# davnords/octic-vits

Measured on AMD Instinct MI355X. Metric: images/sec Hybrid Octic ViT-H/14 224² bf16 train step @1/2/4/8 MI355X, higher is better.
Workload: dtype bf16; 1 GPU; hybrid_deit_huge_patch14 (16 octic + 16 standard blocks, drop_path 0.5) DeiT-III train step: bf16-autocast fwd + bwd + LAMB + EMA, 224x224, batch 64/GPU (BASELINE configs[1]), data parallel over 1 GPU(s); global_batch=64, per_gpu_batch=64, accum_steps=1, parallelism=dp1, library_gemm_table=True, launch=hipGraph replay (whole step)

## Files before the change

include/octic_hip.h:

```cpp
#ifndef OCTIC_HIP_H
#define OCTIC_HIP_H

#include <stdint.h>

#ifdef __cplusplus
extern "C" {
#endif

#define OCTIC_ABI_VERSION 20

enum { OCTIC_F32 = 0, OCTIC_BF16 = 1, OCTIC_U8 = 2  };

enum {
  OCTIC_OK = 0,
  OCTIC_ESHAPE = -1,
  OCTIC_EALIGN = -2,
  OCTIC_EDTYPE = -3,
  OCTIC_ENULL = -4,
  OCTIC_EWORKSPACE = -5
};

typedef struct {
  void* ptr[5];
  int64_t ld[5];
// ... 100 lines not shown
int octic_linear_d8_ring_order_dropped(int ngroups, const int* items, const int* ksteps, int slots_per_xcd, const int* n_chunks,
                                       const unsigned char* dead_long, const unsigned char* dead_short, int* out_group,
                                       int* out_item, int* out_dead);

int octic_linear_d8_wgrad_has_colsum(int cin, int cout, int dtype);
enum {
  OCTIC_WGRAD_RING = 0,
  OCTIC_WGRAD_TILED = 1
};
int octic_linear_d8_wgrad_plan(int64_t M, int cin, int cout, int dtype, int out[4]);
int64_t octic_linear_d8_wgrad_workspace_bytes(int cin, int cout, int splits);
int octic_linear_d8_wgrad_splits(int64_t M, int cin, int cout);
int octic_linear_d8_wgrad_tile(int64_t M, int cin, int cout);
int octic_linear_d8_wgrad(const octic_view* x, const octic_view* dy, int64_t M, int cin, int cout, int dtype,
                          float* workspace, int splits, void* stream);
int octic_linear_d8_wgrad_finish(const float* workspace, int splits, int cin, int cout,
                                 const float* const w32[5], const float* const cs[5], const float* bias,
                                 const float* dysum, float* const dw[5], float* const dcs[5], float* dbias,
                                 void* stream);
typedef struct octic_wgrad_finish_job {
  const float* workspace;
  const float* w32[5];
  const float* cs[5];
  const float* bias;
  const float* dysum;
  float* dw[5];
  float* dcs[5];
  float* dbias;
  int splits, cin, cout, has_cs;
} octic_wgrad_finish_job;
// ... 448 lines not shown
```

octic_vits_amd/_lib.py:

```python
import ctypes
import os
import re

HERE = os.path.dirname(os.path.abspath(__file__))
LIB_PATH = os.environ.get("OCTIC_LIB") or os.path.join(HERE, "liboctic_hip.so")
HEADER_PATH = os.path.join(HERE, "..", "include", "octic_hip.h")

F32, BF16, U8 = 0, 1, 2
ABI_VERSION = 20
(ROUTE_DENSE_TILE, ROUTE_DENSE_SPLIT, ROUTE_WGRAD_SLABS, ROUTE_WGRAD_TILE, ROUTE_LINEAR_RING, ROUTE_RING_EVEN,
 ROUTE_ATTN_LEGACY, ROUTE_ATTN_ONLINE, ROUTE_ATTN_BWD_PAIR, ROUTE_DENSE_IMAGE, ROUTE_DENSE_CLS2, ROUTE_ATTN_STREAM) = range(12)

DENSE_ADAPT_WIDE, DENSE_ADAPT_NARROW = 16, 32
DENSE_IMAGE_ALWAYS, DENSE_IMAGE_CLS_APART, DENSE_IMAGE_NEVER = 4, 8, 16

(ATTN_FWD_PERSIST, ATTN_FWD_A80_ONESHOT, ATTN_FWD_A80_ONLINE, ATTN_FWD_RESIDENT, ATTN_FWD_STREAM, ATTN_FWD_F32) = range(6)
ATTN_BWD_SINGLE, ATTN_BWD_PAIR, ATTN_BWD_STREAM, ATTN_BWD_F32 = range(4)
LINEAR_WREG, LINEAR_RING, LINEAR_CLASSIC = range(3)
WGRAD_RING, WGRAD_TILED = range(2)
DENSE_F32_NT, DENSE_F32_NN, DENSE_F32_TN = range(3)

c_i64, c_int, c_float, c_void_p = ctypes.c_int64, ctypes.c_int, ctypes.c_float, ctypes.c_void_p
c_double = ctypes.c_double

# ... 31 lines not shown
    "octic_linear_d8_fwd": (c_int, [VP, c_void_p, c_void_p, VP, VP, c_void_p, c_i64, c_void_p, c_i64, c_int, c_int,
                                    c_int, c_int, c_void_p]),
    "octic_linear_d8_fwd_skip": (c_int, [VP, c_void_p, c_void_p, VP, VP, c_void_p, c_i64, c_void_p, c_i64, c_int, c_int,
                                         c_int, c_int, c_void_p, c_i64, c_void_p]),
    "octic_linear_d8_fwd_dropped": (c_int, [VP, c_void_p, c_void_p, VP, VP, c_void_p, c_i64, c_void_p, c_i64, c_int, c_int,
                                            c_int, c_int, c_void_p, c_i64, c_void_p]),
    "octic_linear_d8_tile_n": (c_int, [c_i64, c_int, c_int]),
    "octic_linear_d8_plan": (c_int, [c_i64, c_int, c_int, c_int, c_int, c_int, ctypes.POINTER(c_int)]),
    "octic_linear_d8_ring_order": (c_int, [c_void_p, c_void_p, c_void_p, c_int, c_void_p, c_void_p]),
    "octic_linear_d8_ring_order_dropped": (c_int, [c_int, c_void_p, c_void_p, c_int, c_void_p, c_void_p, c_void_p, c_void_p,
                                                   c_void_p, c_void_p]),
    "octic_linear_d8_wgrad_tile": (c_int, [c_i64, c_int, c_int]),
    "octic_linear_d8_wgrad_workspace_bytes": (c_i64, [c_int, c_int, c_int]),
    "octic_linear_d8_wgrad_splits": (c_int, [c_i64, c_int, c_int]),
    "octic_linear_d8_wgrad": (c_int, [VP, VP, c_i64, c_int, c_int, c_int, c_void_p, c_int, c_void_p]),
    "octic_linear_d8_wgrad_finish": (c_int, [c_void_p, c_int, c_int, c_int, c_void_p, c_void_p, c_void_p, c_void_p,
                                             c_void_p, c_void_p, c_void_p, c_void_p]),
    "octic_linear_d8_wgrad_finish_batch": (c_int, [c_void_p, c_int, c_void_p]),
    "octic_linear_d8_wgrad_has_colsum": (c_int, [c_int, c_int, c_int]),
    "octic_linear_d8_wgrad_plan": (c_int, [c_i64, c_int, c_int, c_int, ctypes.POINTER(c_int)]),
    "octic_lamb_workspace_floats": (c_i64, [c_int, c_int]),
    "octic_lamb_step": (c_int, [c_void_p] * 10 + [c_int, c_int, c_void_p, c_float, c_float, c_float, c_float, c_float,
                                                  c_int, c_float, c_void_p, c_void_p]),
    "octic_adamw_step": (c_int, [c_void_p] * 10 + [c_int, c_int, c_void_p, c_float, c_float, c_float, c_float, c_float,
                                                   c_int, c_float, c_void_p, c_void_p]),
    "octic_lamb_step_hp": (c_int, [c_void_p] * 10 + [c_int, c_int, c_void_p, c_void_p, c_float, c_float, c_float, c_float,
                                                     c_int, c_void_p, c_void_p, c_void_p]),
    "octic_adamw_step_hp": (c_int, [c_void_p] * 10 + [c_int, c_int, c_void_p, c_void_p, c_float, c_float, c_float, c_float,
                                                      c_int, c_void_p, c_void_p, c_void_p]),
    "octic_dense_blocks": (c_int, [c_i64]),
# ... 283 lines not shown
```

octic_vits_amd/csrc/wgrad.hip:

```cpp
#include <stdlib.h>
#include "octic_common.hpp"

namespace octic {

struct WgGroup {
  const char* x;
  int64_t x_ld;
  const char* dy;
  int64_t dy_ld;
  int64_t rows;
  int K, N;
  int pair;
  int k_tiles, n_tiles;
  int wg_begin;
  int splits;
  int64_t slab_off;
  float* colsum;
};
struct WgArgs {
  WgGroup g[5];
  int ngroups;
  int wgs;
  int64_t slab_elems;
  float* slabs;
};

template <typename T> struct WElem;
template <> struct WElem<float> { static constexpr int EPC = 4; static constexpr int BMR = 32; };
template <> struct WElem<bf16> { static constexpr int EPC = 8; static constexpr int BMR = 64; };

template <typename TIN, int TT>
__global__ __launch_bounds__(256) void wgrad_kernel(WgArgs args) {
  constexpr int EPC = WElem<TIN>::EPC;
  constexpr int BMR = WElem<TIN>::BMR;
  constexpr int BW = 32 * TT;
  constexpr int CPR = BW / EPC;
  constexpr int RS = BW * (int)sizeof(TIN) + 16;
  constexpr int TILE = BMR * RS;
  extern __shared__ __attribute__((aligned(16))) char lds[];
// ... 135 lines not shown
#ifndef OCTIC_WG_STAGES
#define OCTIC_WG_STAGES 3
#endif
constexpr int kWgS = OCTIC_WG_STAGES, kWgR = 32;
constexpr int kWgTile = kWgR * 320;
constexpr int kWgStage = 2 * kWgTile;
__device__ __attribute__((aligned(256))) unsigned char g_wg_zero[512];

__device__ inline void wg_wait_tiles(int ahead) {
  if (ahead <= 0) asm volatile("s_waitcnt vmcnt(0)" ::: "memory");
  else if (ahead == 1) asm volatile("s_waitcnt vmcnt(5)" ::: "memory");
  else if (ahead == 2) asm volatile("s_waitcnt vmcnt(10)" ::: "memory");
  else asm volatile("s_waitcnt vmcnt(15)" ::: "memory");
}

__global__ __launch_bounds__(256, 2) void wgrad_ring_kernel(WgArgs args) {
  constexpr int TT = 5, BW = 160;
  extern __shared__ __attribute__((aligned(16))) char lds[];
  const int nwg = gridDim.x, bid = blockIdx.x;
  const int xcd = bid & 7, q8 = nwg >> 3, r8 = nwg & 7;
  const int lid = (xcd < r8 ? xcd * (q8 + 1) : r8 * (q8 + 1) + (xcd - r8) * q8) + (bid >> 3);
  int gi = 0;
#pragma unroll
  for (int i = 1; i < 5; ++i)
    if (i < args.ngroups && lid >= args.g[i].wg_begin) gi = i;
  const WgGroup& G = args.g[gi];
  const int gt = G.k_tiles * G.n_tiles;
  const int rel = lid - G.wg_begin;
  const int split = rel / gt, lt = rel - split * gt;
  const int kt = lt / G.n_tiles, nt = lt - kt * G.n_tiles;
  const int k0 = kt * BW, n0 = nt * BW;
  const int K = G.K, N = G.N;
  int64_t chunk = (G.rows + G.splits - 1) / G.splits;
  chunk = (chunk + kWgR - 1) / kWgR * kWgR;
  const int64_t r0 = (int64_t)split * chunk;
  const int64_t r1 = r0 + chunk < G.rows ? r0 + chunk : G.rows;
  const int nsteps = r0 < r1 ? (int)((r1 - r0 + kWgR - 1) / kWgR) : 0;

  const int tid = threadIdx.x, lane = tid & 63, wid = tid >> 6;
  const int wk = wid & 1, wn = wid >> 1;
  const int fr = lane & 15, kg = lane >> 4;

  const char* src[5];
  int64_t inc[5];
  int row_in_tile[5], cbyte[5], ldst[5];
#pragma unroll
  for (int j = 0; j < 5; ++j) {
    const int q = wid + 4 * j;
    const bool isY = q >= 10;
    const int qq = isY ? q - 10 : q;
    const int o = qq * 1024 + lane * 16;
    const int row = o / 320;
    const int cpos = (o - row * 320) >> 4;
    const int c = ((row & 8) ? cpos + 18 : cpos) % 20;
    const int64_t mm = r0 + row;
    const int64_t ld = isY ? G.dy_ld : G.x_ld;
    const int width = isY ? N : K;
    const int64_t ro = G.pair ? (mm >> 1) * ld + (mm & 1) * (int64_t)width : mm * ld;
    src[j] = (isY ? G.dy : G.x) + (ro + (isY ? n0 : k0)) * 2 + c * 16;
    inc[j] = (G.pair ? 16 : 32) * ld * 2;
    row_in_tile[j] = row;
    cbyte[j] = c * 16;
    ldst[j] = (isY ? kWgTile : 0) + qq * 1024;
  }
  int l_step = 0, l_stage = 0;
  auto issue = [&]() {
    const unsigned st = lds_offset(lds) + l_stage * kWgStage;
    const bool tail = (int64_t)(l_step + 1) * kWgR > r1 - r0;
#pragma unroll
    for (int j = 0; j < 5; ++j) {
      const char* p = src[j];
      if (tail && r0 + (int64_t)l_step * kWgR + row_in_tile[j] >= r1) p = (const char*)g_wg_zero + cbyte[j];
      dma16_to_lds(st + ldst[j], p);
      src[j] += inc[j];
    }
    l_stage = l_stage == kWgS - 1 ? 0 : l_stage + 1;
    ++l_step;
  };

  f32x4 acc[TT][TT];
#pragma unroll
  for (int i = 0; i < TT; ++i)
#pragma unroll
    for (int j = 0; j < TT; ++j) acc[i][j] = f32x4{0, 0, 0, 0};
  const bool do_cs = G.colsum != nullptr && kt == 0 && wk == 0;
  f32x4 accs[TT];
#pragma unroll
  for (int j = 0; j < TT; ++j) accs[j] = f32x4{0, 0, 0, 0};
  const bf16 one = (bf16)1.0f;
  const bf16x8 ones = {one, one, one, one, one, one, one, one};

  const int frow = kg * 8 + (fr >> 2);
  const int rot = (kg & 1) * 2;
  int offa[TT], offb[TT];
#pragma unroll
  for (int i = 0; i < TT; ++i) {
    const int ca = wk * 10 + i * 2 + ((fr & 3) >> 1), cb = wn * 10 + i * 2 + ((fr & 3) >> 1);
    offa[i] = frow * 320 + ((ca + rot) % 20) * 16 + (fr & 1) * 8;
    offb[i] = kWgTile + frow * 320 + ((cb + rot) % 20) * 16 + (fr & 1) * 8;
  }

#pragma unroll
  for (int pz = 0; pz < kWgS - 1; ++pz)
    if (pz < nsteps) issue();
  int c_stage = 0;
  for (int sidx = 0; sidx < nsteps; ++sidx) {
    const int left = nsteps - 1 - sidx;
    wg_wait_tiles(left < kWgS - 2 ? left : kWgS - 2);
    __builtin_amdgcn_s_barrier();
    if (sidx + kWgS - 1 < nsteps) issue();
    const char* base = lds + c_stage * kWgStage;
    c_stage = c_stage == kWgS - 1 ? 0 : c_stage + 1;
    typedef __attribute__((ext_vector_type(8))) short s16x8;
    bf16x8 af[TT], bfr[TT];
#pragma unroll
    for (int i = 0; i < TT; ++i) {
// ... 144 lines not shown
    a.g[i].n_tiles = (a.g[i].N + BW - 1) / BW;
    a.g[i].wg_begin = t;
    t += a.g[i].k_tiles * a.g[i].n_tiles * a.g[i].splits;
  }
  a.wgs = t;
  constexpr size_t smem = (size_t)2 * 2 * WElem<TIN>::BMR * (BW * sizeof(TIN) + 16);
  static DeviceOnce once;
  if (once.first()) {
    (void)hipFuncSetAttribute((const void*)wgrad_kernel<TIN, TT>, hipFuncAttributeMaxDynamicSharedMemorySize, (int)smem);
    (void)hipGetLastError();
  }
  wgrad_kernel<TIN, TT><<<t, 256, smem, s>>>(a);
  return launch_status();
}

inline int launch_wgrad_ring(WgArgs& a, hipStream_t s) {
  int t = 0;
  for (int i = 0; i < a.ngroups; ++i) {
    a.g[i].k_tiles = a.g[i].K / 160;
    a.g[i].n_tiles = a.g[i].N / 160;
    a.g[i].wg_begin = t;
    t += a.g[i].k_tiles * a.g[i].n_tiles * a.g[i].splits;
  }
  a.wgs = t;
  static DeviceOnce once;
  if (kWgS * kWgStage > 64 * 1024 && once.first()) {
    (void)hipFuncSetAttribute((const void*)wgrad_ring_kernel, hipFuncAttributeMaxDynamicSharedMemorySize, kWgS * kWgStage);
    (void)hipGetLastError();
  }
  wgrad_ring_kernel<<<t, 256, kWgS * kWgStage, s>>>(a);
  return launch_status();
}

#ifndef OCTIC_WG_TARGET
#define OCTIC_WG_TARGET 512.0
#endif
struct WgPlan {
  int kernel;
  int tt;
  int splits;
};
inline WgPlan wgrad_plan(const WgArgs& a, int dtype) {
  WgPlan p = {dtype == OCTIC_BF16 ? OCTIC_WGRAD_RING : OCTIC_WGRAD_TILED, pick_tt(a), 1};
  for (int i = 0; i < a.ngroups; ++i)
    if ((a.g[i].K % 160) || (a.g[i].N % 160)) p.kernel = OCTIC_WGRAD_TILED;
// ... 50 lines not shown
}

int octic_linear_d8_wgrad_has_colsum(int cin, int cout, int dtype) {
  int out[4];
  return octic_linear_d8_wgrad_plan(1, cin, cout, dtype, out) == OCTIC_OK && out[3];
}
int octic_linear_d8_wgrad_tile(int64_t M, int cin, int cout) {
  int out[4];
  return octic_linear_d8_wgrad_plan(M, cin, cout, OCTIC_F32, out) == OCTIC_OK ? out[1] : 0;
}
int octic_linear_d8_wgrad_splits(int64_t M, int cin, int cout) {
  int out[4];
  return octic_linear_d8_wgrad_plan(M, cin, cout, OCTIC_F32, out) == OCTIC_OK ? out[2] : 1;
}

int octic_linear_d8_wgrad(const octic_view* x, const octic_view* dy, int64_t M, int cin, int cout, int dtype,
                          float* workspace, int splits, void* stream) {
  int e;
  if ((e = check_c_dt(cin, dtype)) || (e = check_c_dt(cout, dtype))) return e;
  if ((e = check_view(x, cin, dtype)) || (e = check_view(dy, cout, dtype))) return e;
  if (!workspace) return OCTIC_ENULL;
  if (M <= 0 || splits <= 0) return OCTIC_ESHAPE;
  WgArgs a = {};
  a.slab_elems = linear_slab_elems(cin, cout);
  a.slabs = workspace;
  d8_group_table(a, M, cin, cout);
  for (int gidx = 0; gidx < 5; ++gidx) {
    const int irrep = d8_group_irrep(gidx);
    const bool isE = irrep == 4;
    WgGroup& g = a.g[gidx];
    g.x = (const char*)x->ptr[irrep];
    g.x_ld = x->ld[irrep];
    g.dy = (const char*)dy->ptr[irrep];
    g.dy_ld = dy->ld[irrep];
    g.splits = group_splits(splits, isE);
    g.slab_off = isE ? (int64_t)4 * cin * cout : (int64_t)irrep * cin * cout;
    g.colsum = irrep == 0 ? workspace + colsum_off_elems(cin, cout, splits) : nullptr;
  }
  if (dtype == OCTIC_F32) return launch_wgrad<float>(a, (hipStream_t)stream);
  if (dtype == OCTIC_BF16) return launch_wgrad<bf16>(a, (hipStream_t)stream);
// ... 108 lines not shown
```

octic_vits_amd/d8_layers.py:

```python
import collections.abc
import math
from itertools import repeat

import torch
import torch.nn as nn
import torch.nn.functional as F

from . import functional as OF
from .d8_utils import SQRT2, SQRT2_OVER_4, convert_5tuple_to_8tuple, convert_8tuple_to_5tuple, expand_lift_kernel, packed_lift_weight
from .functional import Octic, as_packed, compute_dtype


def _ntuple(n):
    def parse(x):
        if isinstance(x, collections.abc.Iterable) and not isinstance(x, str):
            return tuple(x)
        return tuple(repeat(x, n))
    return parse


to_2tuple = _ntuple(2)

drop_path_mask_source = None

# ... 204 lines not shown
        if input_channels % 8 != 0 or output_channels % 8 != 0:
            raise ValueError()
        self.bias = bias
        self.input_channels, self.output_channels = input_channels, output_channels
        ci, co = input_channels // 8, output_channels // 8
        self.lin_A1 = nn.Linear(ci, co, bias=bias)
        self.lin_A2 = nn.Linear(ci, co, bias=False)
        self.lin_B1 = nn.Linear(ci, co, bias=False)
        self.lin_B2 = nn.Linear(ci, co, bias=False)
        self.lin_E = nn.Linear(2 * ci, 2 * co, bias=False)
        self._prep = OF.WeightPrep()

    def weights(self):
        return tuple(getattr(self, "lin_" + n).weight for n in _IRREPS)

    def forward(self, x_batched, resid=None, rs=None, cs=None, next_norm=None, skip_out=None, skip_dx=None, zero_dx=None):
        assert len(x_batched) == 5, "Input should be a 5-tuple"
        xp, cin = as_packed(x_batched)
        if 8 * cin != self.input_channels:
            raise ValueError(f"LinearD8: expected {self.input_channels} channels, got {8 * cin}")
        cout = self.output_channels // 8
        dtype = compute_dtype(xp)
        rps = xp.shape[-2] if xp.dim() >= 2 else 1
        if rs is not None and rs.numel() == xp.numel() // xp.shape[-1] and rs.numel() != xp.shape[0]:
            rps = 1
        cs5 = (None,) * 5 if cs is None else tuple(cs)
        if torch.compiler.is_compiling():
            from . import dispatch as _D
            xq = xp if xp.dtype == dtype else xp.to(dtype)
            fl = self._prep.flat if dtype == torch.bfloat16 else None
            pwb, pwt = fl if fl is not None else (None, None)
            y = torch.ops.octic.linear_d8(xq, *self.weights(), self.lin_A1.bias, resid, rs, *cs5, cin, cout, rps, pwb, pwt)
            return Octic(y, cout) if next_norm is None else (Octic(y, cout), None)
        if (next_norm is not None and resid is not None and OF.OCTIC_NEXT_NORM and xp.is_cuda and dtype == torch.bfloat16
                and resid.dtype == torch.float32 and type(next_norm) is LayerNormD8):
            a, beta = next_norm.affine()
            y, yn = OF.LinearD8NormFn.apply(xp, *self.weights(), self.lin_A1.bias, resid, rs, *cs5, cin, cout, rps, dtype,
                                            self._prep, *a, beta, next_norm.eps, skip_dx)
            return Octic(y, cout), Octic(yn, cout)
        y = OF.LinearD8Fn.apply(xp, *self.weights(), self.lin_A1.bias, resid, rs, *cs5, cin, cout, rps, dtype, self._prep,
                                skip_out, skip_dx, zero_dx)
        return Octic(y, cout) if next_norm is None else (Octic(y, cout), None)

    def extra_repr(self) -> str:
        return f"in_features={self.input_channels}, out_features={self.output_channels}, bias={self.bias is not None}"


class AffineD8(nn.Module):

    def __init__(self, dim, bias=True):
        super().__init__()
        if dim % 8 != 0:
            raise ValueError()
        self.alpha_A1 = nn.Parameter(torch.ones(dim // 8))
        self.alpha_A2 = nn.Parameter(torch.ones(dim // 8))
        self.alpha_B1 = nn.Parameter(torch.ones(dim // 8))
# ... 64 lines not shown
    def __init__(self, in_features, hidden_features=None, out_features=None, act_layer=TritonGeluD8, norm_layer=None,
                 bias=True, drop=0.):
        super().__init__()
        out_features = out_features or in_features
        hidden_features = hidden_features or in_features
        bias = to_2tuple(bias)
        drop_probs = to_2tuple(drop)
        self.fc1 = LinearD8(in_features, hidden_features, bias=bias[0])
        self.act = act_layer()
        self.drop1 = DropoutD8(drop_probs[0])
        self.norm = norm_layer(hidden_features) if norm_layer is not None else nn.Identity()
        self.fc2 = LinearD8(hidden_features, out_features, bias=bias[1])
        self.drop2 = DropoutD8(drop_probs[1])

    def _sample_mask(self, xs, resid, rs):
        if not (OF.LINEAR_SKIP_DROPPED and rs is not None and resid is not None and not COMPACT_DROP_PATH
                and type(self.fc1) is LinearD8 and type(self.fc2) is LinearD8 and type(self.act) is TritonGeluD8
                and type(self.norm) is nn.Identity and not self.drop1.active and not self.drop2.active
                and isinstance(xs, Octic) and xs.packed.dim() == 3 and xs.packed.is_cuda):
            return None
        xp = xs.packed
        return OF.linear_skip_scale(rs, xp.shape[1], xp.shape[0] * xp.shape[1])

    def forward(self, xs, resid=None, rs=None, cs=None, next_norm=None):
        mask = self._sample_mask(xs, resid, rs)
        if mask is not None:
            h = self.fc1(xs, skip_out=mask, zero_dx=mask)
            a = Octic(OF.GeluD8PackedFn.apply(h.packed, h.c, mask, h.packed.shape[1]), h.c)
            return self.fc2(a, resid=resid, rs=rs, cs=cs, next_norm=next_norm, skip_dx=mask)
        xs = self.norm(self.drop1(self.act(self.fc1(xs))))
        if self.drop2.active or resid is None:
            out = _tail(self.drop2(self.fc2(xs)), resid, rs, cs)
            return out if next_norm is None else (out, None)
        return self.fc2(xs, resid=resid, rs=rs, cs=cs, next_norm=next_norm)


def _tail(ys, resid, rs, cs):
    if resid is None:
        return ys
    yp, c = as_packed(ys)
    yp = yp.to(resid.dtype)
    if cs is not None:
        yp = yp * torch.cat(tuple(cs) + (cs[4],)).to(yp.dtype)
    if rs is not None:
        yp = yp * rs.view(-1, *([1] * (yp.dim() - 1))).to(yp.dtype)
# ... 235 lines not shown
        B, T, H = xp.shape[0], xp.shape[1], self.num_heads
        if OF.skip_scale(rs, B) is None or OF.linear_skip_scale(rs, T, B * T) is None:
            return None
        if not OF.ops.attn_skips_dropped(B, T, 8 * (c // H), ld=(3 * 8 * c, 8 * c, 3 * 8 * c)):
            return None
        return rs

    def forward(self, xs, resid=None, rs=None, cs=None, next_norm=None):
        xp, c = as_packed(xs)
        if xp.dim() != 3:
            raise ValueError("AttentionD8 expects [B, N, C] irreps")
        drop = self.attn_drop.p if self.training else 0.
        rag = OF.RAGGED
        gemm_mask = self._gemm_mask(xp, c, resid, rs, drop, rag)
        zero_dx = rs if self._plain_packed(xp, c, resid, rs, drop, rag) else None
        qkv = self.qkv(xs if isinstance(xs, Octic) else Octic(xp, c), skip_out=gemm_mask, zero_dx=zero_dx)
        if rag is not None and rag.matches(xp):
            from . import ragged as _R
            if not (OF.ATTN_PACKED and drop == 0. and qkv.packed.is_cuda
                    and all(OF.ops.attn_packed_ok(T, c, self.num_heads, qkv.packed.dtype) for _, T, _ in rag.sets)):
                raise RuntimeError("AttentionD8: a ragged row tensor needs the packed attention kernels (bf16, head_dim 80 / 64)")
            on = Octic(_R.AttnPackedRaggedFn.apply(qkv.packed, rag, self.num_heads, c, (8 * c // self.num_heads) ** -0.5), c)
        elif (OF.ATTN_PACKED and drop == 0. and qkv.packed.is_cuda
                and OF.ops.attn_packed_ok(qkv.packed.shape[1], c, self.num_heads, qkv.packed.dtype)):
            if torch.compiler.is_compiling():
                from . import dispatch as _D
                on = Octic(torch.ops.octic.attn_packed(qkv.packed, self.num_heads, c, (8 * c // self.num_heads) ** -0.5)[0], c)
            else:
                on = Octic(OF.AttnPackedFn.apply(qkv.packed, self.num_heads, c, (8 * c // self.num_heads) ** -0.5,
                                                 None if (COMPACT_DROP_PATH or resid is None) else rs), c)
        else:
# ... 168 lines not shown
```

octic_vits_amd/functional.py:

```python
import os

import torch

from . import ops


class Octic(tuple):

    def __new__(cls, packed: torch.Tensor, c: int):
        self = super().__new__(cls, ops.split_packed(packed, c))
        self.packed, self.c = packed, c
        return self


def as_packed(xs):
    if isinstance(xs, Octic):
        return xs.packed, xs.c
    if len(xs) != 5:
        raise AssertionError("Input should be a 5-tuple")
    c = xs[0].shape[-1]
    if xs[4].shape[-2:] != (2, 2 * c):
        raise ValueError(f"E irrep must be [..., 2, {2 * c}], got {tuple(xs[4].shape)}")
    return torch.cat([xs[0], xs[1], xs[2], xs[3], xs[4].flatten(-2)], dim=-1), c

# ... 195 lines not shown
    ops._require_cuda(x)
    x_in_dtype = x.dtype
    if x.dtype != dtype:
        x = ops.cast_rowscale(_c(x.float()), None, 1, dtype, cin)
    x = _c(x)
    wb, wt = prep.get(w5, cs5, dtype, cin, cout)
    M = x.numel() // (8 * cin)
    y = torch.empty(x.shape[:-1] + (8 * cout,), dtype=out_dtype, device=x.device)
    b32 = None if bias is None else _c(bias.detach().float())
    cs32 = None if cs5 is None else [_c(s.detach().float()) for s in cs5]
    rs32 = None if rs is None else _c(rs.float())
    ctx.lin = (cin, cout, rps, dtype, cs5 is not None, bias is not None, x_in_dtype, wt)
    return x, wb, M, y, b32, cs32, rs32


def _linear_d8_grads(ctx, x, g, w5, cs32, b32, ss_dx, z_dx=None):
    cin, cout, rps, dtype, has_cs, has_bias, x_in_dtype, wt = ctx.lin
    M = x.numel() // (8 * cin)
    gv, xv = ops.pview(g, cout), ops.pview(x, cin)
    dx = None
    if ctx.needs_input_grad[0]:
        dx = torch.empty(x.shape, dtype=dtype, device=x.device)
        ops.linear_fwd(gv, wt, None, ops.pview(dx, cin), M, cout, cin, dtype, dtype, x, sample_scale=ss_dx, skip_rps=rps,
                       dropped=z_dx, dropped_rps=rps)
        if dx.dtype != x_in_dtype:
            dx = dx.to(x_in_dtype)
    dysum = ops.colsum_a1(gv, M, cout, dtype, x) if (has_bias and not ops.wgrad_has_colsum(cin, cout, dtype)) else None
    w32 = [_c(w.detach().float()) for w in w5] if has_cs else None
    f32_masters = all(w.dtype == torch.float32 for w in w5)
    dw, dcs, dbias = ops.linear_wgrad(xv, gv, M, cin, cout, dtype, x, w32=w32, cs5=cs32, bias=b32, dysum=dysum,
                                      want_bias=has_bias, may_defer=f32_masters, wparams=w5 if f32_masters else None)
    if not f32_masters:
        dw = [d.to(w.dtype) for d, w in zip(dw, w5)]
    return dx, dw, dbias, (dcs if has_cs else [None] * 5)


class LinearD8Fn(torch.autograd.Function):

    @staticmethod
    def forward(ctx, x, wA1, wA2, wB1, wB2, wE, bias, resid, rs, sA1, sA2, sB1, sB2, sE, cin, cout, rps, dtype, prep,
                skip_out=None, skip_dx=None, zero_dx=None):
        w5 = (wA1, wA2, wB1, wB2, wE)
        cs5 = None if sA1 is None else (sA1, sA2, sB1, sB2, sE)
        fused = resid is not None
        out_dtype = resid.dtype if fused else dtype
        handed = x
        x, wb, M, y, b32, cs32, rs32 = _linear_d8_fwd_prep(ctx, x, w5, cs5, bias, rs, cin, cout, rps, dtype, out_dtype, prep)
        rv = ops.pview(_c(resid), cout) if fused else None
        plain = not fused and rs32 is None and cs32 is None
        ss_out = linear_skip_scale(skip_out, rps, M) if plain else None
        dropped = ring_skip_scale(rs32, rps, M) if fused else None
        ops.linear_fwd(ops.pview(x, cin), wb, b32, ops.pview(y, cout), M, cin, cout, dtype, out_dtype, x,
                       resid_v=rv, rs=rs32, rps=rps, cs5=cs32, sample_scale=ss_out, skip_rps=rps, dropped=dropped, dropped_rps=rps)
        ss_dx = linear_skip_scale(skip_dx, rps, M)
        z_dx = ring_skip_scale(zero_dx, rps, M) if (plain and ss_dx is None) else None
        row_skip_fill(handed, row_skip_scale(zero_dx, rps, M) if (plain and ss_dx is None) else None, rps, M)
        ctx.save_for_backward(x, rs32, b32, ss_dx, z_dx, *w5, *(cs32 or []))
        ctx.fused = fused
        return y

    @staticmethod
    def backward(ctx, dy):
        cin, cout, rps, dtype, has_cs = ctx.lin[:5]
        x, rs32, b32, ss_dx, z_dx, *rest = ctx.saved_tensors
        w5, cs32 = rest[:5], (rest[5:] if has_cs else None)
        dy = _c(dy)
        if ctx.fused or rs32 is not None or dy.dtype != dtype:
            g = ops.cast_rowscale(_c(dy.float()), rs32, rps, dtype, cout)
        else:
            g = dy
        dx, dw, dbias, dcs = _linear_d8_grads(ctx, x, g, w5, cs32, b32, ss_dx, z_dx)
        return (dx, *dw, dbias, dy if ctx.fused else None, None, *dcs, None, None, None, None, None, None, None, None)


class LinearD8NormFn(torch.autograd.Function):

    @staticmethod
    def forward(ctx, x, wA1, wA2, wB1, wB2, wE, bias, resid, rs, sA1, sA2, sB1, sB2, sE, cin, cout, rps, dtype, prep,
                a1, a2, b1, b2, ae, beta, eps, skip_dx=None):
        w5 = (wA1, wA2, wB1, wB2, wE)
        cs5 = None if sA1 is None else (sA1, sA2, sB1, sB2, sE)
        x, wb, M, y, b32, cs32, rs32 = _linear_d8_fwd_prep(ctx, x, w5, cs5, bias, rs, cin, cout, rps, dtype, resid.dtype, prep)
        ops.linear_fwd(ops.pview(x, cin), wb, b32, ops.pview(y, cout), M, cin, cout, dtype, resid.dtype, x,
                       resid_v=ops.pview(_c(resid), cout), rs=rs32, rps=rps, cs5=cs32, dropped=ring_skip_scale(rs32, rps, M),
                       dropped_rps=rps)
        alpha = None if a1 is None else [_c(t.float()) for t in (a1, a2, b1, b2, ae)]
        yn, stats = ops.layernorm_fwd(y, alpha, None if beta is None else _c(beta.float()), eps, dtype, cout)
        ctx.save_for_backward(x, rs32, b32, y, stats, linear_skip_scale(skip_dx, rps, M), *w5, *(cs32 or []), *(alpha or []))
        ctx.has_affine, ctx.has_beta = alpha is not None, beta is not None
        ctx.set_materialize_grads(False)
        row_skip_attach(ctx, yn)
        return y, yn

    @staticmethod
    def backward(ctx, dy, dyn):
        cin, cout, rps, dtype, has_cs = ctx.lin[:5]
        has_affine = ctx.has_affine
        x, rs32, b32, y, stats, ss_dx, *rest = ctx.saved_tensors
        w5 = rest[:5]
        cs32 = rest[5:10] if has_cs else None
        alpha = rest[(10 if has_cs else 5):] if has_affine else None
        M = x.numel() // (8 * cin)
        dal, dbeta, g = [None] * 5, None, None
        if dyn is not None:
            dres = None if dy is None else _c(dy.float())
            gn = _c(dyn)
            ns, nrps = row_skip_get(ctx, M)
            mine = dres is not None and STREAM_GRADS.take(dres)
            if ops.layernorm_bwd_cast_ok(gn, y, cout) and dtype == torch.bfloat16:
                dy, dal_, dbeta, g = ops.layernorm_bwd_cast(gn, y, stats, alpha, dres, cout, rs32, rps,
                                                            want_param_grads=has_affine, sample_scale=ns, rows_per_sample=nrps,
                                                            inplace=mine and ns is not None)
            else:
                dy, dal_, dbeta = ops.layernorm_bwd(gn, y, stats, alpha, dres, cout, want_param_grads=has_affine,
                                                    sample_scale=ns, rows_per_sample=nrps)
            dal = dal_ if dal_ is not None else dal
            STREAM_GRADS.offer(dy)
        dy = _c(dy)
        if g is None:
            g = ops.cast_rowscale(_c(dy.float()), rs32, rps, dtype, cout)
        dx, dw, dbias, dcs = _linear_d8_grads(ctx, x, g, w5, cs32, b32, ss_dx)
        return (dx, *dw, dbias, dy, None, *dcs, None, None, None, None, None, *dal, dbeta if ctx.has_beta else None, None, None)


class PackHeadsFn(torch.autograd.Function):

    @staticmethod
    def forward(ctx, qkv, H, c):
        B, T = qkv.shape[0], qkv.shape[1]
        ctx.meta = (B, T, H, c)
        q, k, v = ops.pack_heads(_c(qkv), B, T, H, c, 3)
        return q, k, v

    @staticmethod
    def backward(ctx, gq, gk, gv):
        B, T, H, c = ctx.meta
        return ops.unpack_heads([gq, gk, gv], B, T, H, c), None, None
# ... 76 lines not shown
DENSE_IMAGE_DROPPED = _skip_from_env("OCTIC_DENSE_IMAGE_SKIP")


def dense_skip_scale(rs, rps, M, rows_to=None):
    return whole_sample_mask(rs, rps, M, rows_to) if DENSE_NT_SKIP_DROPPED else None


LINEAR_SKIP_DROPPED = _skip_from_env("OCTIC_LINEAR_SKIP")


def linear_skip_scale(rs, rps, M, rows_to=None):
    return whole_sample_mask(rs, rps, M, rows_to) if LINEAR_SKIP_DROPPED else None


RING_SKIP_DROPPED = _skip_from_env("OCTIC_RING_SKIP")


def ring_skip_scale(rs, rps, M):
    return linear_skip_scale(rs, rps, M) if RING_SKIP_DROPPED else None


ROW_SKIP_DROPPED = _skip_from_env("OCTIC_ROW_SKIP")


def row_skip_scale(rs, rps, M, rows_to=None):
    return whole_sample_mask(rs, rps, M, rows_to) if ROW_SKIP_DROPPED else None


class RowSkipSlot:
    __slots__ = ("scale", "rps", "rows", "fills")
# ... 897 lines not shown
```

octic_vits_amd/ops.py:

```python
import ctypes
import operator

import torch

from . import _lib
from ._lib import BF16, F32, OcticView, PtrArray5, check, lib

_DT = {torch.float32: F32, torch.bfloat16: BF16}
_DTN = {torch.float32: "f32", torch.bfloat16: "bf16"}


class KernelTimer:

    def __init__(self):
        self.on = False
        self.records = []
        self.overhead_us = 0.0

    def enable(self):
        self.on, self.records = True, []
        pairs = []
        for _ in range(64):
            e0, e1 = torch.cuda.Event(enable_timing=True), torch.cuda.Event(enable_timing=True)
            e0.record()
# ... 369 lines not shown
        nbytes = M * 8 * cin * es + M * 8 * cout * eo * (2 if resid_v is not None else 1) + 8 * cin * cout * es
        fused = int(resid_v is not None or rs is not None or cs5 is not None)
        KERNEL_TIMER.stop(t, linear_kernel_name(cin, cout, dtype, out_dtype, fused, M), nbytes, 24.0 * M * cin * cout)


def linear_kernel_name(cin, cout, dtype, out_dtype, fused, M):
    kernel, _, fused, _ = _lib.plan("octic_linear_d8_plan", M, cin, cout, dt_code(dtype), dt_code(out_dtype), int(fused))
    if kernel == _lib.LINEAR_WREG:
        return f"linear_d8_wreg_kernel<{_DTN[out_dtype]},{fused}>"
    if kernel == _lib.LINEAR_RING:
        return f"linear_d8_ring_kernel<{_DTN[dtype]},{_DTN[out_dtype]},{fused}>"
    return f"linear_d8_kernel<{_DTN[dtype]},{_DTN[out_dtype]}>"


def linear_wgrad(xv, dyv, M, cin, cout, dtype, ref, w32=None, cs5=None, bias=None, dysum=None, want_bias=False,
                 may_defer=True, wparams=None):
    L = lib()
    dev = ref.device
    kernel, tile, splits, _ = _lib.plan("octic_linear_d8_wgrad_plan", M, cin, cout, dt_code(dtype))
    ws = torch.empty(L.octic_linear_d8_wgrad_workspace_bytes(cin, cout, splits) // 4, dtype=torch.float32, device=dev)
    t = KERNEL_TIMER.start()
    check(L.octic_linear_d8_wgrad(ctypes.byref(xv), ctypes.byref(dyv), M, cin, cout, dt_code(dtype), _p(ws), splits,
                                  _stream(ref)))
    if t is not None:
        es = 2 if dtype == torch.bfloat16 else 4
        name = "wgrad_ring_kernel<bf16>" if kernel == _lib.WGRAD_RING else f"wgrad_kernel<{_DTN[dtype]},{tile // 32}>"
        slab = (splits + (splits + 1) // 2) * 4 * cin * cout * 4
        KERNEL_TIMER.stop(t, name, M * 8 * (cin + cout) * es + slab, 24.0 * M * cin * cout)
    shapes = [(cout, cin)] * 4 + [(2 * cout, 2 * cin)]
    dests = [grad_dest(w, sh) for w, sh in zip(wparams, shapes)] if wparams is not None else [None] * 5
    dw = [d if d is not None else torch.empty(sh, dtype=torch.float32, device=dev) for d, sh in zip(dests, shapes)]
    dcs = None
    if cs5 is not None:
        dcs = [torch.empty(cout, dtype=torch.float32, device=dev) for _ in range(4)]
        dcs.append(torch.empty(2 * cout, dtype=torch.float32, device=dev))
    dbias = torch.empty(cout, dtype=torch.float32, device=dev) if want_bias else None
    landed = [w for w, d in zip(wparams, dests) if d is not None] if wparams is not None else []
    if may_defer and DEFERRED_FINISHES.enabled and DEFERRED_FINISHES.slabs_too and _in_backward():
# ... 1848 lines not shown
```

Before: 1296 images/s.

## Skip drop-path-dropped samples in octic linear wgrad ring kernel

Adds a SKIP variant of the wgrad ring kernel. It builds an LDS bitmask of K-steps that contain at least one live (non-dropped) sample and splits only those live steps across the existing splits. The Python side passes the drop-path sample scale into the weight-gradient path for fc1/qkv linears, so rows whose upstream gradient is zero are never loaded or multiplied. With drop_path 0.5, about half the rows are zero and the wgrad GEMM work should shrink. In exchange, each workgroup does a prologue mask build and scan, and load balance depends on the mask at runtime.

```diff
diff --git a/include/octic_hip.h b/include/octic_hip.h
--- a/include/octic_hip.h
+++ b/include/octic_hip.h
@@ -138,6 +138,10 @@
 int octic_linear_d8_wgrad_tile(int64_t M, int cin, int cout);
 int octic_linear_d8_wgrad(const octic_view* x, const octic_view* dy, int64_t M, int cin, int cout, int dtype,
                           float* workspace, int splits, void* stream);
+int octic_linear_d8_wgrad_skip(const octic_view* x, const octic_view* dy, int64_t M, int cin, int cout, int dtype,
+                               float* workspace, int splits, const float* sample_scale, int rows_per_sample, void* stream);
+int octic_linear_d8_wgrad_order_dropped(int64_t M, int cin, int cout, int dtype, int splits, const float* sample_scale,
+                                        int rows_per_sample, int cap, int* out_group, int* out_split, int* out_step);
 int octic_linear_d8_wgrad_finish(const float* workspace, int splits, int cin, int cout,
                                  const float* const w32[5], const float* const cs[5], const float* bias,
                                  const float* dysum, float* const dw[5], float* const dcs[5], float* dbias,
diff --git a/octic_vits_amd/_lib.py b/octic_vits_amd/_lib.py
--- a/octic_vits_amd/_lib.py
+++ b/octic_vits_amd/_lib.py
@@ -69,6 +69,9 @@
     "octic_linear_d8_wgrad_workspace_bytes": (c_i64, [c_int, c_int, c_int]),
     "octic_linear_d8_wgrad_splits": (c_int, [c_i64, c_int, c_int]),
     "octic_linear_d8_wgrad": (c_int, [VP, VP, c_i64, c_int, c_int, c_int, c_void_p, c_int, c_void_p]),
+    "octic_linear_d8_wgrad_skip": (c_int, [VP, VP, c_i64, c_int, c_int, c_int, c_void_p, c_int, c_void_p, c_int, c_void_p]),
+    "octic_linear_d8_wgrad_order_dropped": (c_int, [c_i64, c_int, c_int, c_int, c_int, c_void_p, c_int, c_int, c_void_p,
+                                                    c_void_p, c_void_p]),
     "octic_linear_d8_wgrad_finish": (c_int, [c_void_p, c_int, c_int, c_int, c_void_p, c_void_p, c_void_p, c_void_p,
                                              c_void_p, c_void_p, c_void_p, c_void_p]),
     "octic_linear_d8_wgrad_finish_batch": (c_int, [c_void_p, c_int, c_void_p]),
diff --git a/octic_vits_amd/csrc/wgrad.hip b/octic_vits_amd/csrc/wgrad.hip
--- a/octic_vits_amd/csrc/wgrad.hip
+++ b/octic_vits_amd/csrc/wgrad.hip
@@ -23,6 +23,8 @@
   int wgs;
   int64_t slab_elems;
   float* slabs;
+  const float* sample_scale;
+  int rows_per_sample;
 };
 
 template <typename T> struct WElem;
@@ -188,6 +190,24 @@
   else asm volatile("s_waitcnt vmcnt(15)" ::: "memory");
 }
 
+constexpr int kWgLiveWords = 64;
+__host__ __device__ inline int wg_group_steps(int64_t rows) { return (int)((rows + kWgR - 1) / kWgR); }
+__host__ __device__ inline void wg_step_samples(int t, int64_t rows, int pair, int rows_per_sample, int& b0, int& b1) {
+  const int64_t m0 = (int64_t)t * kWgR;
+  const int64_t m1 = m0 + kWgR < rows ? m0 + kWgR : rows;
+  b0 = (int)((m0 >> pair) / rows_per_sample);
+  b1 = (int)(((m1 - 1) >> pair) / rows_per_sample);
+}
+__host__ __device__ inline bool wg_step_live(const float* sample_scale, int t, int64_t rows, int pair, int rows_per_sample) {
+  int b0, b1;
+  wg_step_samples(t, rows, pair, rows_per_sample, b0, b1);
+  bool live = false;
+  for (int b = b0; b <= b1; ++b) live |= sample_scale[b] != 0.f;
+  return live;
+}
+__host__ __device__ inline int wg_share_begin(int L, int s, int S) { return (int)((int64_t)L * s / S); }
+
+template <bool SKIP>
 __global__ __launch_bounds__(256, 2) void wgrad_ring_kernel(WgArgs args) {
   constexpr int TT = 5, BW = 160;
   extern __shared__ __attribute__((aligned(16))) char lds[];
@@ -207,13 +227,46 @@
   const int K = G.K, N = G.N;
   int64_t chunk = (G.rows + G.splits - 1) / G.splits;
   chunk = (chunk + kWgR - 1) / kWgR * kWgR;
-  const int64_t r0 = (int64_t)split * chunk;
-  const int64_t r1 = r0 + chunk < G.rows ? r0 + chunk : G.rows;
-  const int nsteps = r0 < r1 ? (int)((r1 - r0 + kWgR - 1) / kWgR) : 0;
+  const int64_t r0 = SKIP ? 0 : (int64_t)split * chunk;
+  const int64_t r1 = (!SKIP && r0 + chunk < G.rows) ? r0 + chunk : G.rows;
+  int nsteps = r0 < r1 ? (int)((r1 - r0 + kWgR - 1) / kWgR) : 0;
 
   const int tid = threadIdx.x, lane = tid & 63, wid = tid >> 6;
   const int wk = wid & 1, wn = wid >> 1;
   const int fr = lane & 15, kg = lane >> 4;
+
+  constexpr int PRE = 5;
+  [[maybe_unused]] const int gsteps = nsteps;
+  [[maybe_unused]] unsigned long long* live_words = nullptr;
+  [[maybe_unused]] float pre_a[PRE], pre_b[PRE];
+  [[maybe_unused]] int nwords = 0;
+  [[maybe_unused]] auto live_request = [&](int w, float& fa, float& fb) {
+    const int t = w * 64 + lane;
+    int b0, b1;
+    wg_step_samples(t < gsteps ? t : gsteps - 1, G.rows, G.pair, args.rows_per_sample, b0, b1);
+    fa = args.sample_scale[b0];
+    fb = args.sample_scale[b1];
+  };
+  [[maybe_unused]] auto live_store = [&](int w, float fa, float fb) {
+    const int t = w * 64 + lane;
+    bool live = false;
+    if (t < gsteps) {
+      int b0, b1;
+      wg_step_samples(t, G.rows, G.pair, args.rows_per_sample, b0, b1);
+      live = fa != 0.f || fb != 0.f;
+      for (int b = b0 + 1; b < b1; ++b) live |= args.sample_scale[b] != 0.f;
+    }
+    const unsigned long long m = __ballot(live);
+    if (lane == 0) live_words[w] = m;
+  };
+  if constexpr (SKIP) {
+    __shared__ unsigned long long wg_live[kWgLiveWords];
+    live_words = wg_live;
+    nwords = (gsteps + 63) >> 6;
+#pragma unroll
+    for (int i = 0; i < PRE; ++i)
+      if (wid + 4 * i < nwords) live_request(wid + 4 * i, pre_a[i], pre_b[i]);
+  }
 
   const char* src[5];
   int64_t inc[5];
@@ -238,15 +291,39 @@
     ldst[j] = (isY ? kWgTile : 0) + qq * 1024;
   }
   int l_step = 0, l_stage = 0;
+  [[maybe_unused]] int live_wi = 0;
+  [[maybe_unused]] unsigned long long live_w = 0;
+  [[maybe_unused]] auto next_live = [&]() {
+    while (live_w == 0) {
+      ++live_wi;
+      const unsigned long long v = live_words[live_wi];
+      live_w = ((unsigned long long)(unsigned)__builtin_amdgcn_readfirstlane((int)(v >> 32)) << 32) |
+               (unsigned)__builtin_amdgcn_readfirstlane((int)v);
+    }
+    const int j = __builtin_ctzll(live_w);
+    live_w &= live_w - 1;
+    return (live_wi << 6) + j;
+  };
   auto issue = [&]() {
     const unsigned st = lds_offset(lds) + l_stage * kWgStage;
-    const bool tail = (int64_t)(l_step + 1) * kWgR > r1 - r0;
-#pragma unroll
-    for (int j = 0; j < 5; ++j) {
-      const char* p = src[j];
-      if (tail && r0 + (int64_t)l_step * kWgR + row_in_tile[j] >= r1) p = (const char*)g_wg_zero + cbyte[j];
-      dma16_to_lds(st + ldst[j], p);
-      src[j] += inc[j];
+    if constexpr (SKIP) {
+      const int t = next_live();
+      const bool tail = (int64_t)(t + 1) * kWgR > G.rows;
+#pragma unroll
+      for (int j = 0; j < 5; ++j) {
+        const char* p = src[j] + (int64_t)t * inc[j];
+        if (tail && (int64_t)t * kWgR + row_in_tile[j] >= G.rows) p = (const char*)g_wg_zero + cbyte[j];
+        dma16_to_lds(st + ldst[j], p);
+      }
+    } else {
+      const bool tail = (int64_t)(l_step + 1) * kWgR > r1 - r0;
+#pragma unroll
+      for (int j = 0; j < 5; ++j) {
+        const char* p = src[j];
+        if (tail && r0 + (int64_t)l_step * kWgR + row_in_tile[j] >= r1) p = (const char*)g_wg_zero + cbyte[j];
+        dma16_to_lds(st + ldst[j], p);
+        src[j] += inc[j];
+      }
     }
     l_stage = l_stage == kWgS - 1 ? 0 : l_stage + 1;
     ++l_step;
@@ -274,6 +351,35 @@
     offb[i] = kWgTile + frow * 320 + ((cb + rot) % 20) * 16 + (fr & 1) * 8;
   }
 
+  if constexpr (SKIP) {
+#pragma unroll
+    for (int i = 0; i < PRE; ++i)
+      if (wid + 4 * i < nwords) live_store(wid + 4 * i, pre_a[i], pre_b[i]);
+    for (int w = wid + 4 * PRE; w < nwords; w += 4) {
+      float fa, fb;
+      live_request(w, fa, fb);
+      live_store(w, fa, fb);
+    }
+    __syncthreads();
+    const unsigned long long mine = lane < nwords ? live_words[lane] : 0ull;
+    const int pc = __popcll(mine);
+    int incl = pc;
+#pragma unroll
+    for (int d = 1; d < 64; d <<= 1) {
+      const int v = __shfl_up(incl, d);
+      if (lane >= d) incl += v;
+    }
+    const int L = __builtin_amdgcn_readfirstlane(__shfl(incl, 63));
+    const int lo = wg_share_begin(L, split, G.splits), hi = wg_share_begin(L, split + 1, G.splits);
+    nsteps = hi - lo;
+    const int wi = __builtin_amdgcn_readfirstlane(__popcll(__ballot(incl <= lo)));
+    const int below = __builtin_amdgcn_readfirstlane(__shfl(incl - pc, wi & 63));
+    unsigned long long w0 = ((unsigned long long)(unsigned)__builtin_amdgcn_readfirstlane(__shfl((int)(mine >> 32), wi & 63)) << 32) |
+                            (unsigned)__builtin_amdgcn_readfirstlane(__shfl((int)mine, wi & 63));
+    for (int i = below; i < lo && nsteps > 0; ++i) w0 &= w0 - 1;
+    live_wi = wi;
+    live_w = nsteps > 0 ? w0 : 0ull;
+  }
 #pragma unroll
   for (int pz = 0; pz < kWgS - 1; ++pz)
     if (pz < nsteps) issue();
@@ -448,6 +554,13 @@
   return launch_status();
 }
 
+inline bool wgrad_ring_masked(const WgArgs& a) {
+  if (!a.sample_scale) return false;
+  for (int i = 0; i < a.ngroups; ++i)
+    if (wg_group_steps(a.g[i].rows) > kWgLiveWords * 64) return false;
+  return true;
+}
+
 inline int launch_wgrad_ring(WgArgs& a, hipStream_t s) {
   int t = 0;
   for (int i = 0; i < a.ngroups; ++i) {
@@ -459,10 +572,12 @@
   a.wgs = t;
   static DeviceOnce once;
   if (kWgS * kWgStage > 64 * 1024 && once.first()) {
-    (void)hipFuncSetAttribute((const void*)wgrad_ring_kernel, hipFuncAttributeMaxDynamicSharedMemorySize, kWgS * kWgStage);
+    (void)hipFuncSetAttribute((const void*)wgrad_ring_kernel<false>, hipFuncAttributeMaxDynamicSharedMemorySize, kWgS * kWgStage);
+    (void)hipFuncSetAttribute((const void*)wgrad_ring_kernel<true>, hipFuncAttributeMaxDynamicSharedMemorySize, kWgS * kWgStage);
     (void)hipGetLastError();
   }
-  wgrad_ring_kernel<<<t, 256, kWgS * kWgStage, s>>>(a);
+  if (wgrad_ring_masked(a)) wgrad_ring_kernel<true><<<t, 256, kWgS * kWgStage, s>>>(a);
+  else wgrad_ring_kernel<false><<<t, 256, kWgS * kWgStage, s>>>(a);
   return launch_status();
 }
 
@@ -543,16 +658,62 @@
   return octic_linear_d8_wgrad_plan(M, cin, cout, OCTIC_F32, out) == OCTIC_OK ? out[2] : 1;
 }
 
+static int wg_mask_status(const float* sample_scale, int rows_per_sample, int64_t M) {
+  if (!sample_scale) return OCTIC_OK;
+  if (rows_per_sample <= 0 || M % rows_per_sample) return OCTIC_ESHAPE;
+  return ((uintptr_t)sample_scale & 3) ? OCTIC_EALIGN : OCTIC_OK;
+}
+
 int octic_linear_d8_wgrad(const octic_view* x, const octic_view* dy, int64_t M, int cin, int cout, int dtype,
                           float* workspace, int splits, void* stream) {
+  return octic_linear_d8_wgrad_skip(x, dy, M, cin, cout, dtype, workspace, splits, nullptr, 0, stream);
+}
+
+int octic_linear_d8_wgrad_order_dropped(int64_t M, int cin, int cout, int dtype, int splits, const float* sample_scale,
+                                        int rows_per_sample, int cap, int* out_group, int* out_split, int* out_step) {
+  int e;
+  if ((e = check_c_dt(cin, dtype)) || (e = check_c_dt(cout, dtype))) return e;
+  if (M <= 0 || splits <= 0 || cap < 0) return OCTIC_ESHAPE;
+  if (!sample_scale || !out_group || !out_split || !out_step) return OCTIC_ENULL;
+  if ((e = wg_mask_status(sample_scale, rows_per_sample, M))) return e;
+  WgArgs a = {};
+  d8_group_table(a, M, cin, cout);
+  a.sample_scale = sample_scale;
+  if (wgrad_plan(a, dtype).kernel != OCTIC_WGRAD_RING || !wgrad_ring_masked(a)) return OCTIC_ESHAPE;
+  int n = 0;
+  for (int gidx = 0; gidx < 5; ++gidx) {
+    const WgGroup& g = a.g[gidx];
+    const int S = group_splits(splits, gidx == 0), T = wg_group_steps(g.rows);
+    int L = 0;
+    for (int t = 0; t < T; ++t) L += wg_step_live(sample_scale, t, g.rows, g.pair, rows_per_sample);
+    int rank = 0, s = 0;
+    for (int t = 0; t < T; ++t) {
+      if (!wg_step_live(sample_scale, t, g.rows, g.pair, rows_per_sample)) continue;
+      while (rank >= wg_share_begin(L, s + 1, S)) ++s;
+      if (n >= cap) return OCTIC_ESHAPE;
+      out_group[n] = gidx;
+      out_split[n] = s;
+      out_step[n] = t;
+      ++n;
+      ++rank;
+    }
+  }
+  return n;
+}
+
+int octic_linear_d8_wgrad_skip(const octic_view* x, const octic_view* dy, int64_t M, int cin, int cout, int dtype,
+                               float* workspace, int splits, const float* sample_scale, int rows_per_sample, void* stream) {
   int e;
   if ((e = check_c_dt(cin, dtype)) || (e = check_c_dt(cout, dtype))) return e;
   if ((e = check_view(x, cin, dtype)) || (e = check_view(dy, cout, dtype))) return e;
   if (!workspace) return OCTIC_ENULL;
   if (M <= 0 || splits <= 0) return OCTIC_ESHAPE;
+  if ((e = wg_mask_status(sample_scale, rows_per_sample, M))) return e;
   WgArgs a = {};
   a.slab_elems = linear_slab_elems(cin, cout);
   a.slabs = workspace;
+  a.sample_scale = sample_scale;
+  a.rows_per_sample = rows_per_sample;
   d8_group_table(a, M, cin, cout);
   for (int gidx = 0; gidx < 5; ++gidx) {
     const int irrep = d8_group_irrep(gidx);
diff --git a/octic_vits_amd/d8_layers.py b/octic_vits_amd/d8_layers.py
--- a/octic_vits_amd/d8_layers.py
+++ b/octic_vits_amd/d8_layers.py
@@ -242,7 +242,8 @@
     def weights(self):
         return tuple(getattr(self, "lin_" + n).weight for n in _IRREPS)
 
-    def forward(self, x_batched, resid=None, rs=None, cs=None, next_norm=None, skip_out=None, skip_dx=None, zero_dx=None):
+    def forward(self, x_batched, resid=None, rs=None, cs=None, next_norm=None, skip_out=None, skip_dx=None, zero_dx=None,
+                zero_dy=None):
         assert len(x_batched) == 5, "Input should be a 5-tuple"
         xp, cin = as_packed(x_batched)
         if 8 * cin != self.input_channels:
@@ -253,6 +254,7 @@
         if rs is not None and rs.numel() == xp.numel() // xp.shape[-1] and rs.numel() != xp.shape[0]:
             rps = 1
         cs5 = (None,) * 5 if cs is None else tuple(cs)
+        zero_dy = None if COMPACT_DROP_PATH else (rs if rs is not None else zero_dy)
         if torch.compiler.is_compiling():
             from . import dispatch as _D
             xq = xp if xp.dtype == dtype else xp.to(dtype)
@@ -264,10 +266,10 @@
                 and resid.dtype == torch.float32 and type(next_norm) is LayerNormD8):
             a, beta = next_norm.affine()
             y, yn = OF.LinearD8NormFn.apply(xp, *self.weights(), self.lin_A1.bias, resid, rs, *cs5, cin, cout, rps, dtype,
-                                            self._prep, *a, beta, next_norm.eps, skip_dx)
+                                            self._prep, *a, beta, next_norm.eps, skip_dx, zero_dy)
             return Octic(y, cout), Octic(yn, cout)
         y = OF.LinearD8Fn.apply(xp, *self.weights(), self.lin_A1.bias, resid, rs, *cs5, cin, cout, rps, dtype, self._prep,
-                                skip_out, skip_dx, zero_dx)
+                                skip_out, skip_dx, zero_dx, zero_dy)
         return Octic(y, cout) if next_norm is None else (Octic(y, cout), None)
 
     def extra_repr(self) -> str:
@@ -362,21 +364,25 @@
         self.drop2 = DropoutD8(drop_probs[1])
 
     def _sample_mask(self, xs, resid, rs):
-        if not (OF.LINEAR_SKIP_DROPPED and rs is not None and resid is not None and not COMPACT_DROP_PATH
-                and type(self.fc1) is LinearD8 and type(self.fc2) is LinearD8 and type(self.act) is TritonGeluD8
-                and type(self.norm) is nn.Identity and not self.drop1.active and not self.drop2.active
-                and isinstance(xs, Octic) and xs.packed.dim() == 3 and xs.packed.is_cuda):
+        if not (OF.LINEAR_SKIP_DROPPED and self._plain_chain(xs, resid, rs)):
             return None
         xp = xs.packed
         return OF.linear_skip_scale(rs, xp.shape[1], xp.shape[0] * xp.shape[1])
 
+    def _plain_chain(self, xs, resid, rs):
+        return (rs is not None and resid is not None and not COMPACT_DROP_PATH
+                and type(self.fc1) is LinearD8 and type(self.fc2) is LinearD8 and type(self.act) is TritonGeluD8
+                and type(self.norm) is nn.Identity and not self.drop1.active and not self.drop2.active
+                and isinstance(xs, Octic) and xs.packed.dim() == 3 and xs.packed.is_cuda)
+
     def forward(self, xs, resid=None, rs=None, cs=None, next_norm=None):
         mask = self._sample_mask(xs, resid, rs)
+        zero_dy = rs if (self._plain_chain(xs, resid, rs) and not torch.compiler.is_compiling()) else None
         if mask is not None:
-            h = self.fc1(xs, skip_out=mask, zero_dx=mask)
+            h = self.fc1(xs, skip_out=mask, zero_dx=mask, zero_dy=zero_dy)
             a = Octic(OF.GeluD8PackedFn.apply(h.packed, h.c, mask, h.packed.shape[1]), h.c)
             return self.fc2(a, resid=resid, rs=rs, cs=cs, next_norm=next_norm, skip_dx=mask)
-        xs = self.norm(self.drop1(self.act(self.fc1(xs))))
+        xs = self.norm(self.drop1(self.act(self.fc1(xs, zero_dy=zero_dy) if zero_dy is not None else self.fc1(xs))))
         if self.drop2.active or resid is None:
             out = _tail(self.drop2(self.fc2(xs)), resid, rs, cs)
             return out if next_norm is None else (out, None)
@@ -642,7 +648,7 @@
         rag = OF.RAGGED
         gemm_mask = self._gemm_mask(xp, c, resid, rs, drop, rag)
         zero_dx = rs if self._plain_packed(xp, c, resid, rs, drop, rag) else None
-        qkv = self.qkv(xs if isinstance(xs, Octic) else Octic(xp, c), skip_out=gemm_mask, zero_dx=zero_dx)
+        qkv = self.qkv(xs if isinstance(xs, Octic) else Octic(xp, c), skip_out=gemm_mask, zero_dx=zero_dx, zero_dy=zero_dx)
         if rag is not None and rag.matches(xp):
             from . import ragged as _R
             if not (OF.ATTN_PACKED and drop == 0. and qkv.packed.is_cuda
diff --git a/octic_vits_amd/functional.py b/octic_vits_amd/functional.py
--- a/octic_vits_amd/functional.py
+++ b/octic_vits_amd/functional.py
@@ -233,7 +233,7 @@
     return x, wb, M, y, b32, cs32, rs32
 
 
-def _linear_d8_grads(ctx, x, g, w5, cs32, b32, ss_dx, z_dx=None):
+def _linear_d8_grads(ctx, x, g, w5, cs32, b32, ss_dx, z_dx=None, ss_dw=None):
     cin, cout, rps, dtype, has_cs, has_bias, x_in_dtype, wt = ctx.lin
     M = x.numel() // (8 * cin)
     gv, xv = ops.pview(g, cout), ops.pview(x, cin)
@@ -248,7 +248,8 @@
     w32 = [_c(w.detach().float()) for w in w5] if has_cs else None
     f32_masters = all(w.dtype == torch.float32 for w in w5)
     dw, dcs, dbias = ops.linear_wgrad(xv, gv, M, cin, cout, dtype, x, w32=w32, cs5=cs32, bias=b32, dysum=dysum,
-                                      want_bias=has_bias, may_defer=f32_masters, wparams=w5 if f32_masters else None)
+                                      want_bias=has_bias, may_defer=f32_masters, wparams=w5 if f32_masters else None,
+                                      sample_scale=ss_dw if f32_masters else None, rows_per_sample=rps)
     if not f32_masters:
         dw = [d.to(w.dtype) for d, w in zip(dw, w5)]
     return dx, dw, dbias, (dcs if has_cs else [None] * 5)
@@ -258,7 +259,7 @@
 
     @staticmethod
     def forward(ctx, x, wA1, wA2, wB1, wB2, wE, bias, resid, rs, sA1, sA2, sB1, sB2, sE, cin, cout, rps, dtype, prep,
-                skip_out=None, skip_dx=None, zero_dx=None):
+                skip_out=None, skip_dx=None, zero_dx=None, zero_dy=None):
         w5 = (wA1, wA2, wB1, wB2, wE)
         cs5 = None if sA1 is None else (sA1, sA2, sB1, sB2, sE)
         fused = resid is not None
@@ -274,29 +275,30 @@
         ss_dx = linear_skip_scale(skip_dx, rps, M)
         z_dx = ring_skip_scale(zero_dx, rps, M) if (plain and ss_dx is None) else None
         row_skip_fill(handed, row_skip_scale(zero_dx, rps, M) if (plain and ss_dx is None) else None, rps, M)
-        ctx.save_for_backward(x, rs32, b32, ss_dx, z_dx, *w5, *(cs32 or []))
+        ss_dw = linear_wgrad_skip_scale(rs32 if (rs is not None and zero_dy is rs) else zero_dy, rps, M)
+        ctx.save_for_backward(x, rs32, b32, ss_dx, z_dx, ss_dw, *w5, *(cs32 or []))
         ctx.fused = fused
         return y
 
     @staticmethod
     def backward(ctx, dy):
         cin, cout, rps, dtype, has_cs = ctx.lin[:5]
-        x, rs32, b32, ss_dx, z_dx, *rest = ctx.saved_tensors
+        x, rs32, b32, ss_dx, z_dx, ss_dw, *rest = ctx.saved_tensors
         w5, cs32 = rest[:5], (rest[5:] if has_cs else None)
         dy = _c(dy)
         if ctx.fused or rs32 is not None or dy.dtype != dtype:
             g = ops.cast_rowscale(_c(dy.float()), rs32, rps, dtype, cout)
         else:
             g = dy
-        dx, dw, dbias, dcs = _linear_d8_grads(ctx, x, g, w5, cs32, b32, ss_dx, z_dx)
-        return (dx, *dw, dbias, dy if ctx.fused else None, None, *dcs, None, None, None, None, None, None, None, None)
+        dx, dw, dbias, dcs = _linear_d8_grads(ctx, x, g, w5, cs32, b32, ss_dx, z_dx, ss_dw)
+        return (dx, *dw, dbias, dy if ctx.fused else None, None, *dcs, None, None, None, None, None, None, None, None, None)
 
 
 class LinearD8NormFn(torch.autograd.Function):
 
     @staticmethod
     def forward(ctx, x, wA1, wA2, wB1, wB2, wE, bias, resid, rs, sA1, sA2, sB1, sB2, sE, cin, cout, rps, dtype, prep,
-                a1, a2, b1, b2, ae, beta, eps, skip_dx=None):
+                a1, a2, b1, b2, ae, beta, eps, skip_dx=None, zero_dy=None):
         w5 = (wA1, wA2, wB1, wB2, wE)
         cs5 = None if sA1 is None else (sA1, sA2, sB1, sB2, sE)
         x, wb, M, y, b32, cs32, rs32 = _linear_d8_fwd_prep(ctx, x, w5, cs5, bias, rs, cin, cout, rps, dtype, resid.dtype, prep)
@@ -305,7 +307,9 @@
                        dropped_rps=rps)
         alpha = None if a1 is None else [_c(t.float()) for t in (a1, a2, b1, b2, ae)]
         yn, stats = ops.layernorm_fwd(y, alpha, None if beta is None else _c(beta.float()), eps, dtype, cout)
-        ctx.save_for_backward(x, rs32, b32, y, stats, linear_skip_scale(skip_dx, rps, M), *w5, *(cs32 or []), *(alpha or []))
+        ss_dw = linear_wgrad_skip_scale(rs32 if (rs is not None and zero_dy is rs) else zero_dy, rps, M)
+        ctx.save_for_backward(x, rs32, b32, y, stats, linear_skip_scale(skip_dx, rps, M), ss_dw, *w5, *(cs32 or []),
+                              *(alpha or []))
         ctx.has_affine, ctx.has_beta = alpha is not None, beta is not None
         ctx.set_materialize_grads(False)
         row_skip_attach(ctx, yn)
@@ -315,7 +319,7 @@
     def backward(ctx, dy, dyn):
         cin, cout, rps, dtype, has_cs = ctx.lin[:5]
         has_affine = ctx.has_affine
-        x, rs32, b32, y, stats, ss_dx, *rest = ctx.saved_tensors
+        x, rs32, b32, y, stats, ss_dx, ss_dw, *rest = ctx.saved_tensors
         w5 = rest[:5]
         cs32 = rest[5:10] if has_cs else None
         alpha = rest[(10 if has_cs else 5):] if has_affine else None
@@ -338,8 +342,9 @@
         dy = _c(dy)
         if g is None:
             g = ops.cast_rowscale(_c(dy.float()), rs32, rps, dtype, cout)
-        dx, dw, dbias, dcs = _linear_d8_grads(ctx, x, g, w5, cs32, b32, ss_dx)
-        return (dx, *dw, dbias, dy, None, *dcs, None, None, None, None, None, *dal, dbeta if ctx.has_beta else None, None, None)
+        dx, dw, dbias, dcs = _linear_d8_grads(ctx, x, g, w5, cs32, b32, ss_dx, ss_dw=ss_dw)
+        return (dx, *dw, dbias, dy, None, *dcs, None, None, None, None, None, *dal, dbeta if ctx.has_beta else None, None, None,
+                None)
 
 
 class PackHeadsFn(torch.autograd.Function):
@@ -446,6 +451,13 @@
 
 
 RING_SKIP_DROPPED = _skip_from_env("OCTIC_RING_SKIP")
+
+
+LINEAR_WGRAD_SKIP_DROPPED = _skip_from_env("OCTIC_LINEAR_WGRAD_SKIP")
+
+
+def linear_wgrad_skip_scale(rs, rps, M):
+    return whole_sample_mask(rs, rps, M) if LINEAR_WGRAD_SKIP_DROPPED else None
 
 
 def ring_skip_scale(rs, rps, M):
diff --git a/octic_vits_amd/ops.py b/octic_vits_amd/ops.py
--- a/octic_vits_amd/ops.py
+++ b/octic_vits_amd/ops.py
@@ -407,14 +407,18 @@
 
 
 def linear_wgrad(xv, dyv, M, cin, cout, dtype, ref, w32=None, cs5=None, bias=None, dysum=None, want_bias=False,
-                 may_defer=True, wparams=None):
+                 may_defer=True, wparams=None, sample_scale=None, rows_per_sample=0):
     L = lib()
     dev = ref.device
     kernel, tile, splits, _ = _lib.plan("octic_linear_d8_wgrad_plan", M, cin, cout, dt_code(dtype))
     ws = torch.empty(L.octic_linear_d8_wgrad_workspace_bytes(cin, cout, splits) // 4, dtype=torch.float32, device=dev)
     t = KERNEL_TIMER.start()
-    check(L.octic_linear_d8_wgrad(ctypes.byref(xv), ctypes.byref(dyv), M, cin, cout, dt_code(dtype), _p(ws), splits,
-                                  _stream(ref)))
+    if sample_scale is None:
+        check(L.octic_linear_d8_wgrad(ctypes.byref(xv), ctypes.byref(dyv), M, cin, cout, dt_code(dtype), _p(ws), splits,
+                                      _stream(ref)))
+    else:
+        check(L.octic_linear_d8_wgrad_skip(ctypes.byref(xv), ctypes.byref(dyv), M, cin, cout, dt_code(dtype), _p(ws), splits,
+                                           _p(sample_scale), int(rows_per_sample), _stream(ref)))
     if t is not None:
         es = 2 if dtype == torch.bfloat16 else 4
         name = "wgrad_ring_kernel<bf16>" if kernel == _lib.WGRAD_RING else f"wgrad_kernel<{_DTN[dtype]},{tile // 32}>"
```

New measurement: 1318 images/s, median of 6. 1.7% higher.
